# maturk/dn-splatter

Hardware: NVIDIA H100
Metric: rendered Mpix/s (fwd+bwd, RGB+depth+normal) (higher is better)
Workload: dtype f32

## Files before the change

### dn_splatter_b200/csrc/ssim.cu

```cuda
#include "common.cuh"

namespace {

constexpr int SS_R = 5;
constexpr int SS_T = 16;
constexpr int SS_H = SS_T + 2 * SS_R;
constexpr int SS_P = 28;
constexpr int SS_C = 3;
constexpr int SS_NT = 256;

__constant__ float c_win[11] = {1.028380357e-03f, 7.598758209e-03f, 3.600077331e-02f, 1.093606874e-01f, 2.130055279e-01f,
                                2.660117149e-01f, 2.130055279e-01f, 1.093606874e-01f, 3.600077331e-02f, 7.598758209e-03f,
                                1.028380357e-03f};

template <bool U8>
__device__ __forceinline__ float ld_gt(const void* img, size_t idx) {
  return U8 ? __fmul_rn((float)((const uint8_t*)img)[idx], 1.0f / 255.0f) : ((const float*)img)[idx];
}

template <int NQ_IN, int NQ_OUT, int NC, typename Make>
__device__ __forceinline__ void hpass(float (*s_in)[SS_C][SS_H][SS_P], float (*s_mid)[SS_C][SS_H][SS_T], int tid, Make make) {
  constexpr int items = NC * SS_H * (SS_T / 2);
  for (int it = tid; it < items; it += SS_NT) {
    const int seg = it % (SS_T / 2), r = (it / (SS_T / 2)) % SS_H, c = it / ((SS_T / 2) * SS_H);
    float in[NQ_IN][12];
#pragma unroll
    for (int q = 0; q < NQ_IN; ++q) {
      const float2* p = reinterpret_cast<const float2*>(&s_in[q][c][r][2 * seg]);
#pragma unroll
      for (int k = 0; k < 6; ++k) { const float2 v = p[k]; in[q][2 * k] = v.x; in[q][2 * k + 1] = v.y; }
    }
    float acc[NQ_OUT][2];
#pragma unroll
    for (int q = 0; q < NQ_OUT; ++q) acc[q][0] = acc[q][1] = 0.f;
#pragma unroll
    for (int k = 0; k < 12; ++k) {
      float v[NQ_OUT];
      float src[NQ_IN];
#pragma unroll
      for (int q = 0; q < NQ_IN; ++q) src[q] = in[q][k];
      make(src, v);
#pragma unroll
      for (int q = 0; q < NQ_OUT; ++q) {
        if (k < 11) acc[q][0] += c_win[k] * v[q];
        if (k > 0) acc[q][1] += c_win[k - 1] * v[q];
      }
    }
#pragma unroll
    for (int q = 0; q < NQ_OUT; ++q) *reinterpret_cast<float2*>(&s_mid[q][c][r][2 * seg]) = make_float2(acc[q][0], acc[q][1]);
  }
}

template <int NQ>
__device__ __forceinline__ void vpass(float (*s_mid)[SS_C][SS_H][SS_T], int c, int col, int g, float out[NQ][4]) {
#pragma unroll
  for (int q = 0; q < NQ; ++q) {
    float v[14];
#pragma unroll
    for (int j = 0; j < 14; ++j) v[j] = s_mid[q][c][4 * g + j][col];
#pragma unroll
    for (int o = 0; o < 4; ++o) {
      float acc = 0.f;
#pragma unroll
      for (int k = 0; k < 11; ++k) acc += c_win[k] * v[o + k];
      out[q][o] = acc;
    }
  }
}

template <bool U8, bool L1, int NC>
__global__ void __launch_bounds__(SS_NT) ssim_fwd_kernel(const float* __restrict__ x, const void* __restrict__ y, int H, int W,
                                                        int C, int c0, float* __restrict__ dmaps, float* __restrict__ sum_out) {
  __shared__ __align__(16) float s_in[2][SS_C][SS_H][SS_P];
  __shared__ __align__(16) float s_mid[5][SS_C][SS_H][SS_T];
  __shared__ float red[SS_NT / 32];
  __shared__ float red_l1[SS_NT / 32];
  const int tid = threadIdx.x;
  constexpr int nc = NC;
  const int i0 = blockIdx.y * SS_T - SS_R, j0 = blockIdx.x * SS_T - SS_R;
  for (int e = tid; e < SS_H * SS_H * NC; e += SS_NT) {
    const int c = e % NC, q = (e / NC) % SS_H, r = e / (NC * SS_H);
    const int i = i0 + r, j = j0 + q;
    float xv = 0.f, yv = 0.f;
    if (i >= 0 && i < H && j >= 0 && j < W) {
      const size_t p = ((size_t)i * W + j) * C + c0 + c;
      xv = x[p];
      yv = ld_gt<U8>(y, p);
    }
    s_in[0][c][r][q] = xv;
    s_in[1][c][r][q] = yv;
  }
  __syncthreads();
  hpass<2, 5, NC>(s_in, s_mid, tid, [](const float* s, float* v) {
    v[0] = s[0]; v[1] = s[1]; v[2] = s[0] * s[0]; v[3] = s[1] * s[1]; v[4] = s[0] * s[1];
  });
  __syncthreads();
  float ssum = 0.f, lsum = 0.f;
  if (tid < nc * SS_T * 4) {
    const int col = tid % SS_T, g = (tid / SS_T) % 4, c = tid / (SS_T * 4);
    float f[5][4];
    vpass<5>(s_mid, c, col, g, f);
    const int j = blockIdx.x * SS_T + col;
    const size_t n = (size_t)H * W * C;
#pragma unroll
    for (int o = 0; o < 4; ++o) {
      const int i = blockIdx.y * SS_T + 4 * g + o;
      const bool interior = (i >= SS_R) && (i < H - SS_R) && (j >= SS_R) && (j < W - SS_R);
      float s = 0.f, d_mu = 0.f, d_xx = 0.f, d_xy = 0.f;
      if (interior) {
        const float C1 = 0.0001f, C2 = 0.0009f;
        const float mx = f[0][o], my = f[1][o];
        const float sx = f[2][o] - mx * mx, sy = f[3][o] - my * my, sxy = f[4][o] - mx * my;
        const float A1 = 2.f * mx * my + C1, A2 = 2.f * sxy + C2, B1 = mx * mx + my * my + C1, B2 = sx + sy + C2;
        const float inv = 1.0f / (B1 * B2);
        s = A1 * A2 * inv;
        d_xx = -s / B2;
        d_xy = 2.f * A1 * inv;
        d_mu = 2.f * my * (A2 - A1) * inv - 2.f * mx * s / B1 + 2.f * mx * s / B2;
      }
      if (i < H && j < W) {
        const size_t p = ((size_t)i * W + j) * C + c0 + c;
        dmaps[p] = d_mu; dmaps[n + p] = d_xx; dmaps[2 * n + p] = d_xy;
        if (L1) lsum += fabsf(s_in[0][c][4 * g + o + SS_R][col + SS_R] - s_in[1][c][4 * g + o + SS_R][col + SS_R]);
      }
      ssum += s;
    }
  }
  ssum = warp_sum(ssum);
  if (L1) lsum = warp_sum(lsum);
  if ((tid & 31) == 0) { red[tid >> 5] = ssum; if (L1) red_l1[tid >> 5] = lsum; }
  __syncthreads();
  if (tid == 0) {
    float t = 0.f, tl = 0.f;
#pragma unroll
    for (int w = 0; w < SS_NT / 32; ++w) { t += red[w]; if (L1) tl += red_l1[w]; }
    if (t != 0.f) atomicAdd(sum_out, t);
    if (L1 && tl != 0.f) atomicAdd(sum_out + 1, tl);
  }
}

__global__ void photometric_finish_kernel(float* out, float lambda, float inv_count_ssim, float inv_count_l1) {
  out[2] = (1.0f - lambda) * (out[1] * inv_count_l1) + lambda * (1.0f - out[0] * inv_count_ssim);
}

template <bool U8, int NC>
__global__ void __launch_bounds__(SS_NT) ssim_bwd_kernel(const float* __restrict__ x, const void* __restrict__ y, int H, int W,
                                                        int C, int c0, const float* __restrict__ dmaps, const float* v_mean,
                                                        float w_ssim, float w_l1, float* __restrict__ v_x) {
  __shared__ __align__(16) float s_in[3][SS_C][SS_H][SS_P];
  __shared__ __align__(16) float s_mid[3][SS_C][SS_H][SS_T];
  const int tid = threadIdx.x;
  constexpr int nc = NC;
  const int i0 = blockIdx.y * SS_T - SS_R, j0 = blockIdx.x * SS_T - SS_R;
  const size_t n = (size_t)H * W * C;
  for (int e = tid; e < SS_H * SS_H * NC; e += SS_NT) {
    const int c = e % NC, q = (e / NC) % SS_H, r = e / (NC * SS_H);
    const int i = i0 + r, j = j0 + q;
    float a = 0.f, b = 0.f, d = 0.f;
    if (i >= 0 && i < H && j >= 0 && j < W) {
      const size_t p = ((size_t)i * W + j) * C + c0 + c;
      a = dmaps[p]; b = dmaps[n + p]; d = dmaps[2 * n + p];
    }
    s_in[0][c][r][q] = a; s_in[1][c][r][q] = b; s_in[2][c][r][q] = d;
  }
  __syncthreads();
  hpass<3, 3, NC>(s_in, s_mid, tid, [](const float* s, float* v) { v[0] = s[0]; v[1] = s[1]; v[2] = s[2]; });
  __syncthreads();
  if (tid < nc * SS_T * 4) {
    const int col = tid % SS_T, g = (tid / SS_T) % 4, c = tid / (SS_T * 4);
    float f[3][4];
    vpass<3>(s_mid, c, col, g, f);
    const int j = blockIdx.x * SS_T + col;
    const float count = (float)(H - 2 * SS_R) * (float)(W - 2 * SS_R) * (float)C;
    const float vm = v_mean ? __ldg(v_mean) : 1.0f;
    const float gsc = vm * w_ssim / count;
    const float gl1 = vm * w_l1 / ((float)H * (float)W * (float)C);
#pragma unroll
    for (int o = 0; o < 4; ++o) {
      const int i = blockIdx.y * SS_T + 4 * g + o;
      if (i < H && j < W) {
        const size_t p = ((size_t)i * W + j) * C + c0 + c;
        const float xv = x[p], yv = ld_gt<U8>(y, p);
        const float d = xv - yv;
        v_x[p] = gsc * (f[0][o] + 2.f * xv * f[1][o] + yv * f[2][o]) + gl1 * ((d > 0.f) ? 1.f : ((d < 0.f) ? -1.f : 0.f));
      }
    }
  }
}

}

template <bool L1>
static int launch_ssim_fwd(const float* pred, const void* gt, int gt_is_u8, int H, int W, int C, float* dmaps, float* out, cudaStream_t s) {
  const dim3 grid((W + SS_T - 1) / SS_T, (H + SS_T - 1) / SS_T, 1);
  for (int c0 = 0; c0 < C; c0 += SS_C) {
    const int nc = C - c0 < SS_C ? C - c0 : SS_C;
#define DNR_SSIM_FWD(U8, NC) ssim_fwd_kernel<U8, L1, NC><<<grid, SS_NT, 0, s>>>(pred, gt, H, W, C, c0, dmaps, out)
    if (gt_is_u8) { if (nc == 3) DNR_SSIM_FWD(true, 3); else if (nc == 2) DNR_SSIM_FWD(true, 2); else DNR_SSIM_FWD(true, 1); }
    else { if (nc == 3) DNR_SSIM_FWD(false, 3); else if (nc == 2) DNR_SSIM_FWD(false, 2); else DNR_SSIM_FWD(false, 1); }
#undef DNR_SSIM_FWD
    DNR_CHECK_LAUNCH();
  }
  return 0;
}

static int launch_ssim_bwd(const float* pred, const void* gt, int gt_is_u8, int H, int W, int C, const float* dmaps, const float* v,
                           float w_ssim, float w_l1, float* v_pred, cudaStream_t s) {
  const dim3 grid((W + SS_T - 1) / SS_T, (H + SS_T - 1) / SS_T, 1);
  for (int c0 = 0; c0 < C; c0 += SS_C) {
    const int nc = C - c0 < SS_C ? C - c0 : SS_C;
#define DNR_SSIM_BWD(U8, NC) ssim_bwd_kernel<U8, NC><<<grid, SS_NT, 0, s>>>(pred, gt, H, W, C, c0, dmaps, v, w_ssim, w_l1, v_pred)
    if (gt_is_u8) { if (nc == 3) DNR_SSIM_BWD(true, 3); else if (nc == 2) DNR_SSIM_BWD(true, 2); else DNR_SSIM_BWD(true, 1); }
    else { if (nc == 3) DNR_SSIM_BWD(false, 3); else if (nc == 2) DNR_SSIM_BWD(false, 2); else DNR_SSIM_BWD(false, 1); }
#undef DNR_SSIM_BWD
    DNR_CHECK_LAUNCH();
  }
  return 0;
}

extern "C" int dnr_ssim_fwd_ex(const float* pred, const void* gt, int32_t gt_is_u8, int32_t H, int32_t W, int32_t C, float* dmaps,
                               float* sum_out, void* stream) {
  if (!pred || !gt || !dmaps || !sum_out) return DNR_E_NULL;
  if (H <= 2 * SS_R || W <= 2 * SS_R || C <= 0) return DNR_E_SIZE;
  cudaStream_t s = (cudaStream_t)stream;
  DNR_CUDA(cudaMemsetAsync(sum_out, 0, sizeof(float), s));
  return launch_ssim_fwd<false>(pred, gt, gt_is_u8, H, W, C, dmaps, sum_out, s);
}

extern "C" int dnr_photometric_fwd(const float* pred, const void* gt, int32_t gt_is_u8, int32_t H, int32_t W, int32_t C,
                                   float ssim_lambda, float* dmaps, float* out, void* stream) {
  if (!pred || !gt || !dmaps || !out) return DNR_E_NULL;
  if (H <= 2 * SS_R || W <= 2 * SS_R || C <= 0) return DNR_E_SIZE;
  cudaStream_t s = (cudaStream_t)stream;
  DNR_CUDA(cudaMemsetAsync(out, 0, 3 * sizeof(float), s));
  if (const int rc = launch_ssim_fwd<true>(pred, gt, gt_is_u8, H, W, C, dmaps, out, s)) return rc;
  photometric_finish_kernel<<<1, 1, 0, s>>>(out, ssim_lambda, 1.0f / ((float)(H - 2 * SS_R) * (float)(W - 2 * SS_R) * (float)C),
                                            1.0f / ((float)H * (float)W * (float)C));
  DNR_CHECK_LAUNCH();
  return 0;
}

extern "C" int dnr_photometric_bwd(const float* pred, const void* gt, int32_t gt_is_u8, int32_t H, int32_t W, int32_t C,
                                   float ssim_lambda, const float* dmaps, const float* v_main, float* v_pred, void* stream) {
  if (!pred || !gt || !dmaps || !v_pred) return DNR_E_NULL;
  if (H <= 2 * SS_R || W <= 2 * SS_R || C <= 0) return DNR_E_SIZE;
  return launch_ssim_bwd(pred, gt, gt_is_u8, H, W, C, dmaps, v_main, -ssim_lambda, 1.0f - ssim_lambda, v_pred, (cudaStream_t)stream);
}

extern "C" int dnr_ssim_bwd_ex(const float* pred, const void* gt, int32_t gt_is_u8, int32_t H, int32_t W, int32_t C,
                               const float* dmaps, const float* v_mean, float* v_pred, void* stream) {
  if (!pred || !gt || !dmaps || !v_pred) return DNR_E_NULL;
  if (H <= 2 * SS_R || W <= 2 * SS_R || C <= 0) return DNR_E_SIZE;
  return launch_ssim_bwd(pred, gt, gt_is_u8, H, W, C, dmaps, v_mean, 1.0f, 0.0f, v_pred, (cudaStream_t)stream);
}

extern "C" int dnr_ssim_fwd(const float* pred, const float* gt, int32_t H, int32_t W, int32_t C, float* dmaps, float* sum_out,
                            void* stream) {
  return dnr_ssim_fwd_ex(pred, gt, 0, H, W, C, dmaps, sum_out, stream);
}

extern "C" int dnr_ssim_bwd(const float* pred, const float* gt, int32_t H, int32_t W, int32_t C, const float* dmaps,
                            const float* v_mean, float* v_pred, void* stream) {
  return dnr_ssim_bwd_ex(pred, gt, 0, H, W, C, dmaps, v_mean, v_pred, stream);
}
```

### dn_splatter_b200/regularization_strategy.py

```python
from __future__ import annotations

import ctypes as C
from abc import abstractmethod
from typing import Optional

import torch
import torch.nn as nn
import torch.nn.functional as F
from torch import Tensor

from . import _lib as L
from .losses import DepthLoss, DepthLossType, NormalLoss, NormalLossType

_FUSED_DEPTH = {DepthLossType.EdgeAwareLogL1: 1, DepthLossType.LogL1: 2, DepthLossType.L1: 3, DepthLossType.MSE: 4}


def _stream() -> C.c_void_p:
    return C.c_void_p(torch.cuda.current_stream().cuda_stream)


def _shared_holder(*tensors):
    from .rasterize import raster_holder

    hs = [raster_holder(t) for t in tensors if t is not None]
    if not hs or any(h is None for h in hs) or any(h is not hs[0] for h in hs):
        return None
    return hs[0]


class _FusedDNLoss(torch.autograd.Function):

    @staticmethod
    def forward(ctx, pred_depth, pred_normal, gt_depth, gt_normal, gt_img, depth_type: int, depth_lambda: float,
                depth_tolerance: float, use_normal: bool, holder=None, edge_image=None):
        lib = L.load()
        ref = pred_depth if pred_depth is not None else pred_normal
        if ref.device.type != "cuda":
            raise L.DnrError("DNRegularization: the fused regulariser needs CUDA tensors (no CPU path)")
        if depth_type:
            H, W = pred_depth.shape[0], pred_depth.shape[1]
        else:
            H, W = pred_normal.shape[0], pred_normal.shape[1]
        dev = ref.device

        def prep(t, keep_u8=False):
            if t is None:
                return None
            if keep_u8 and t.dtype == torch.uint8:
                return t.detach().to(device=dev).contiguous()
            return t.detach().to(device=dev, dtype=torch.float32).contiguous()

        pd, pn, gd, gi = prep(pred_depth), prep(pred_normal), prep(gt_depth), prep(gt_img)
        gn = prep(gt_normal, keep_u8=True)
        ei = prep(edge_image, keep_u8=True)
        flags = 0
        if gn is not None and gn.dtype == torch.uint8:
            flags |= L.LOSS_NORMAL_U8
        if ei is not None:
            assert ei.dtype == torch.uint8, "edge_image is the raw uint8 image"
            flags |= L.LOSS_EDGE_FROM_IMAGE | L.LOSS_IMG_U8
        partials = torch.empty(12, dtype=torch.float32, device=dev)
        a = L.DnrArgs()
        a.width, a.height = W, H
        a.depth_loss_type, a.use_normal_loss = int(depth_type), int(bool(use_normal))
        a.depth_lambda, a.depth_tolerance = float(depth_lambda), float(depth_tolerance)
        a.loss_flags = flags
        for k, t in dict(out_depth=pd, out_normal=pn, gt_depth=gd, gt_normal=gn, gt_rgb=gi, gt_image=ei,
                         loss_partials=partials).items():
            setattr(a, k, None if t is None else t.data_ptr())
        L.check(lib.dnr_loss_fwd(C.byref(a), _stream()), "dnr_loss_fwd")
        ctx.keep = (pd, pn, gd, gn, gi, ei, partials)
        ctx.fwd_stream = torch.cuda.current_stream()
        ctx.cfg = (W, H, int(depth_type), int(bool(use_normal)), float(depth_lambda), float(depth_tolerance), flags)
        ctx.shapes = (None if pred_depth is None else pred_depth.shape, None if pred_normal is None else pred_normal.shape)
        ctx.holder = holder
        return partials[11].clone()

    @staticmethod
    def backward(ctx, v):
        with torch.cuda.stream(ctx.fwd_stream):
            return _FusedDNLoss._backward(ctx, v)

    @staticmethod
    def _backward(ctx, v):
        lib = L.load()
        pd, pn, gd, gn, gi, ei, partials = ctx.keep
        W, H, depth_type, use_normal, lam, tol, flags = ctx.cfg
        v = v.detach().to(torch.float32).contiguous()
        none9 = (None,) * 9
        if ctx.holder is not None:
            from .rasterize import zero_token

            ctx.holder.setdefault("deferred", {})["reg"] = dict(
                depth_type=depth_type, use_normal=use_normal, depth_lambda=lam, depth_tolerance=tol, gt_depth=gd,
                gt_normal=gn if use_normal else None, gt_rgb=gi, edge_image=ei, loss_partials=partials, v=v)
            vd = zero_token(pd.view(ctx.shapes[0])) if (depth_type and ctx.needs_input_grad[0]) else None
            vn = zero_token(pn.view(ctx.shapes[1])) if (use_normal and ctx.needs_input_grad[1]) else None
            return (vd, vn) + none9
        a = L.DnrArgs()
        a.width, a.height = W, H
        a.depth_loss_type, a.use_normal_loss, a.depth_lambda, a.depth_tolerance = depth_type, use_normal, lam, tol
        a.loss_flags = flags
        for k, t in dict(out_depth=pd, out_normal=pn, gt_depth=gd, gt_normal=gn, gt_rgb=gi, gt_image=ei,
                         loss_partials=partials, v_loss=v).items():
            setattr(a, k, None if t is None else t.data_ptr())
        vd = torch.empty(ctx.shapes[0], dtype=torch.float32, device=v.device) if (depth_type and ctx.needs_input_grad[0]) else None
        vn = torch.empty(ctx.shapes[1], dtype=torch.float32, device=v.device) if (use_normal and ctx.needs_input_grad[1]) else None
        if vd is not None or vn is not None:
            L.check(lib.dnr_loss_bwd(C.byref(a), None if vd is None else vd.data_ptr(),
                                     None if vn is None else vn.data_ptr(), _stream()), "dnr_loss_bwd")
        return (vd, vn) + none9


class _ScaleLoss(torch.autograd.Function):

    @staticmethod
    def forward(ctx, scales):
        lib = L.load()
        if scales.device.type != "cuda":
            raise L.DnrError("scale loss: CUDA tensor required (no CPU path)")
        s = scales.detach().float().contiguous()
        out = torch.empty(1, dtype=torch.float32, device=s.device)
        L.check(lib.dnr_scale_loss_fwd(s.data_ptr(), s.shape[0], out.data_ptr(), _stream()), "dnr_scale_loss_fwd")
        ctx.s = s
        ctx.fwd_stream = torch.cuda.current_stream()
        return out[0].clone()

    @staticmethod
    def backward(ctx, v):
        with torch.cuda.stream(ctx.fwd_stream):
            return _ScaleLoss._backward(ctx, v)

    @staticmethod
    def _backward(ctx, v):
        lib = L.load()
        s = ctx.s
        v = v.detach().float().contiguous()
        g = torch.empty_like(s)
        L.check(lib.dnr_scale_loss_bwd(s.data_ptr(), s.shape[0], v.data_ptr(), g.data_ptr(), _stream()),
                "dnr_scale_loss_bwd")
        return g


class FusedL1(torch.autograd.Function):

    @staticmethod
    def forward(ctx, pred, gt, holder=None):
        lib = L.load()
        if pred.device.type != "cuda" or gt.device != pred.device:
            raise L.DnrError("FusedL1 needs CUDA tensors on one device (no CPU path)")
        p = pred.detach().float().contiguous()
        g = gt.detach().contiguous()
        if g.dtype != torch.uint8:
            g = g.float()
        assert g.numel() == p.numel(), "pred / gt size mismatch"
        out = torch.empty(1, dtype=torch.float32, device=p.device)
        L.check(lib.dnr_l1_fwd(p.data_ptr(), g.data_ptr(), p.numel(), int(g.dtype == torch.uint8), out.data_ptr(), _stream()),
                "dnr_l1_fwd")
        ctx.keep = (p, g)
        ctx.shape = pred.shape
        ctx.fwd_stream = torch.cuda.current_stream()
        ctx.holder = holder
        return out[0].clone()

    @staticmethod
    def backward(ctx, v):
        with torch.cuda.stream(ctx.fwd_stream):
            return FusedL1._backward(ctx, v)

    @staticmethod
    def _backward(ctx, v):
        lib = L.load()
        p, g = ctx.keep
        v = v.detach().float().contiguous()
        if ctx.holder is not None:
            from .rasterize import zero_token

            ctx.holder.setdefault("deferred", {})["l1"] = dict(gt=g, v=v)
            return zero_token(p.view(ctx.shape)), None, None
        vp = torch.empty_like(p)
        L.check(lib.dnr_l1_bwd(p.data_ptr(), g.data_ptr(), p.numel(), int(g.dtype == torch.uint8), v.data_ptr(), vp.data_ptr(),
                               _stream()), "dnr_l1_bwd")
        return vp.view(ctx.shape), None, None


class FusedSSIM(torch.autograd.Function):

    @staticmethod
    def forward(ctx, pred, gt):
        lib = L.load()
        if pred.device.type != "cuda" or gt.device != pred.device:
            raise L.DnrError("FusedSSIM needs CUDA tensors on one device (no CPU path)")
        p = pred.detach().float().contiguous()
        g = gt.detach().contiguous()
        if g.dtype != torch.uint8:
            g = g.float()
        assert p.dim() == 3 and p.shape == g.shape, "pred / gt must both be [H,W,C]"
        H, W, Cn = p.shape
        dmaps = torch.empty((3, H, W, Cn), dtype=torch.float32, device=p.device)
        out = torch.empty(1, dtype=torch.float32, device=p.device)
        L.check(lib.dnr_ssim_fwd_ex(p.data_ptr(), g.data_ptr(), int(g.dtype == torch.uint8), H, W, Cn, dmaps.data_ptr(),
                                    out.data_ptr(), _stream()), "dnr_ssim_fwd_ex")
        ctx.keep = (p, g, dmaps)
        ctx.fwd_stream = torch.cuda.current_stream()
        return out[0] / float((H - 10) * (W - 10) * Cn)

    @staticmethod
    def backward(ctx, v):
        with torch.cuda.stream(ctx.fwd_stream):
            lib = L.load()
            p, g, dmaps = ctx.keep
            v = v.detach().float().contiguous()
            vp = torch.empty_like(p)
            H, W, Cn = p.shape
            L.check(lib.dnr_ssim_bwd_ex(p.data_ptr(), g.data_ptr(), int(g.dtype == torch.uint8), H, W, Cn, dmaps.data_ptr(),
                                        v.data_ptr(), vp.data_ptr(), _stream()), "dnr_ssim_bwd_ex")
            return vp, None


class FusedPhotometric(torch.autograd.Function):

    @staticmethod
    def forward(ctx, pred, gt, ssim_lambda: float):
        lib = L.load()
        if pred.device.type != "cuda" or gt.device != pred.device:
            raise L.DnrError("FusedPhotometric needs CUDA tensors on one device (no CPU path)")
        p = pred.detach().float().contiguous()
        g = gt.detach().contiguous()
        if g.dtype != torch.uint8:
            g = g.float()
        assert p.dim() == 3 and p.shape == g.shape, "pred / gt must both be [H,W,C]"
        H, W, Cn = p.shape
        dmaps = torch.empty((3, H, W, Cn), dtype=torch.float32, device=p.device)
        out = torch.empty(3, dtype=torch.float32, device=p.device)
        L.check(lib.dnr_photometric_fwd(p.data_ptr(), g.data_ptr(), int(g.dtype == torch.uint8), H, W, Cn, float(ssim_lambda),
                                        dmaps.data_ptr(), out.data_ptr(), _stream()), "dnr_photometric_fwd")
        ctx.keep = (p, g, dmaps)
        ctx.lam = float(ssim_lambda)
        ctx.fwd_stream = torch.cuda.current_stream()
        return out[2].clone()

    @staticmethod
    def backward(ctx, v):
        with torch.cuda.stream(ctx.fwd_stream):
            lib = L.load()
            p, g, dmaps = ctx.keep
            v = v.detach().float().contiguous()
            vp = torch.empty_like(p)
            H, W, Cn = p.shape
            L.check(lib.dnr_photometric_bwd(p.data_ptr(), g.data_ptr(), int(g.dtype == torch.uint8), H, W, Cn, ctx.lam,
                                            dmaps.data_ptr(), v.data_ptr(), vp.data_ptr(), _stream()), "dnr_photometric_bwd")
            return vp, None, None


def u8_to_float(img: Tensor, divisor: float = 255.0, clamp_min: float = 0.0) -> Tensor:
    src = img.contiguous()
    dst = torch.empty(src.shape, dtype=torch.float32, device=src.device)
    L.check(L.load().dnr_u8_to_f32(src.data_ptr(), src.numel(), float(divisor), float(clamp_min), dst.data_ptr(), _stream()),
            "dnr_u8_to_f32")
    return dst


class RegularizationStrategy(nn.Module):

    def __init__(self, **kwargs):
        super().__init__()
        self.device_indicator_param = nn.Parameter(torch.empty(0))

    @property
    def device(self):
        return self.device_indicator_param.device

    @abstractmethod
    def get_loss(self, **kwargs):
        """Loss"""

    def forward(self, **kwargs):
        return self.get_loss(**kwargs)

    def get_scale_loss(self, scales):
        return _ScaleLoss.apply(scales)


class DNRegularization(RegularizationStrategy):

    def __init__(self, depth_tolerance: float = 0.1,
                 depth_loss_type: Optional[DepthLossType] = DepthLossType.EdgeAwareLogL1,
                 depth_lambda: float = 0.2, normal_lambda: float = 0.1):
        super().__init__()
        self.depth_tolerance = depth_tolerance
        self.depth_loss_type = depth_loss_type
        self.depth_loss = DepthLoss(self.depth_loss_type)
        self.depth_lambda = depth_lambda
        self.normal_loss_type = NormalLossType.L1
        self.normal_loss = NormalLoss(self.normal_loss_type)
        self.normal_smooth_loss_type = NormalLossType.Smooth
        self.normal_smooth_loss = NormalLoss(self.normal_smooth_loss_type)
        self.normal_lambda = normal_lambda

    def _fusable(self, with_depth: bool) -> bool:
        return (not with_depth) or self.depth_loss_type in _FUSED_DEPTH

    fuse_backward = True
    """Hand the backward of the fused terms to dnr_raster_bwd when the maps are direct raster outputs."""

    def get_loss(self, pred_depth, gt_depth, pred_normal, gt_normal, **kwargs):
        with_depth = self.depth_loss is not None
        with_normal = self.normal_loss is not None
        if self._fusable(with_depth) and (with_depth or with_normal):
            if with_depth and gt_depth is None:
                raise TypeError("use_depth_loss is set but the batch holds no depth (reference: '>' on NoneType)")
            dtype = _FUSED_DEPTH[self.depth_loss_type] if with_depth else 0
            gt_img = kwargs.get("gt_img") if dtype == 1 else None
            edge_image = None
            if dtype == 1 and gt_img is None:
                raise KeyError("gt_img")
            if gt_img is not None and gt_img.dtype == torch.uint8:
                gt_img, edge_image = None, gt_img
            pd, pn = (pred_depth if with_depth else None), (pred_normal if with_normal else None)
            holder = _shared_holder(pd, pn) if self.fuse_backward else None
            loss = _FusedDNLoss.apply(pd, pn, gt_depth if with_depth else None, gt_normal if with_normal else None, gt_img,
                                      dtype, self.depth_lambda, self.depth_tolerance, with_normal, holder, edge_image)
        else:
            if gt_normal is not None and gt_normal.dtype == torch.uint8:
                gt_normal = u8_to_float(gt_normal) if gt_normal.is_cuda else gt_normal.float() / 255.0
            if kwargs.get("gt_img") is not None and kwargs["gt_img"].dtype == torch.uint8:
                gi = kwargs["gt_img"]
                kwargs["gt_img"] = u8_to_float(gi, 255.0, 10 / 255.0) if gi.is_cuda else (gi.float() / 255.0).clamp(min=10 / 255.0)
            loss = 0.0
            if with_depth:
                loss = loss + self.get_depth_loss(pred_depth, gt_depth, **kwargs)
            if with_normal:
                loss = loss + self.get_normal_loss(pred_normal, gt_normal, **kwargs)
        return loss + self.get_scale_loss(scales=kwargs["scales"])

    def get_depth_loss(self, pred_depth, gt_depth, **kwargs):
        valid = gt_depth > self.depth_tolerance
        if self.depth_loss_type in _FUSED_DEPTH:
            gt_img = kwargs.get("gt_img") if self.depth_loss_type == DepthLossType.EdgeAwareLogL1 else None
            return _FusedDNLoss.apply(pred_depth, None, gt_depth, None, gt_img, _FUSED_DEPTH[self.depth_loss_type],
                                      self.depth_lambda, self.depth_tolerance, False)
        if self.depth_loss_type == DepthLossType.PearsonDepth:
            n_valid = valid.sum()
            glob = (self.depth_loss(pred_depth, gt_depth.float()) * n_valid) / n_valid
            local = (DepthLoss(DepthLossType.LocalPearsonDepthLoss)(pred_depth, gt_depth.float()) * n_valid) / n_valid
            d = glob + self.depth_lambda * local
            return d + self.depth_lambda * d
        d = self.depth_loss(pred_depth[valid], gt_depth[valid].float())
        return d + self.depth_lambda * d

    def get_normal_loss(self, pred_normal, gt_normal, **kwargs):
        return _FusedDNLoss.apply(None, pred_normal, None, gt_normal, None, 0, 0.0, self.depth_tolerance, True)


def mean_angular_error(pred: Tensor, gt: Tensor) -> Tensor:
    return torch.arccos(torch.clip((gt * pred).sum(0), -1.0, 1.0))


def find_edges(im: Tensor, threshold: float = 0.01, dilation_itr: int = 1) -> Tensor:
    c = im.shape[0]
    lap = torch.tensor([[0, 1, 0], [1, -4, 1], [0, 1, 0]], dtype=torch.float32, device=im.device)
    lap = lap[None, None].expand(c, 1, 3, 3).contiguous()
    box = torch.ones(c, 1, 3, 3, dtype=torch.float32, device=im.device)
    edges = (F.conv2d((1.0 / (im.float() + 1e-6))[None], lap, padding=1, groups=c) > threshold).float()
    dil = edges
    for _ in range(dilation_itr):
        dil = F.conv2d(dil if c == 1 else edges, box, padding=1, groups=c)
    return dil[0] > 0.0


class AGSMeshRegularization(RegularizationStrategy):

    def __init__(self, depth_tolerance: float = 0.1,
                 depth_loss_type: Optional[DepthLossType] = DepthLossType.EdgeAwareLogL1, depth_lambda: float = 0.2,
                 normal_lambda: float = 0.1, normal_mask_steps: int = 15000, depth_mask_steps: int = 7000):
        super().__init__()
        self.depth_tolerance, self.depth_loss_type = depth_tolerance, depth_loss_type
        self.depth_loss = DepthLoss(self.depth_loss_type)
        self.depth_lambda = depth_lambda
        self.normal_loss_type = NormalLossType.L1
        self.normal_loss = NormalLoss(self.normal_loss_type)
        self.normal_smooth_loss_type = NormalLossType.Smooth
        self.normal_smooth_loss = NormalLoss(self.normal_smooth_loss_type)
        self.normal_lambda = normal_lambda
        self.normal_mask_steps, self.depth_mask_steps = normal_mask_steps, depth_mask_steps
        self.step = 0

    def get_loss(self, step, pred_depth, gt_depth, surf_normal, gt_normal, pred_normal, confidence_map, **kwargs):
        d = self.get_depth_loss(step=step, pred_depth=pred_depth, gt_depth=gt_depth, confidence_map=confidence_map, **kwargs)
        n = self.get_normal_loss(step, surf_normal, gt_normal, pred_normal)
        return d + n + self.get_scale_loss(scales=kwargs["scales"])

    def get_scale_loss(self, scales):
        return torch.min(torch.exp(scales), dim=1, keepdim=True)[0].mean()

    def get_depth_loss(self, step, pred_depth, gt_depth, confidence_map, **kwargs):
        if step >= 7000:
            gt_depth = torch.where(confidence_map > 0, gt_depth, torch.zeros_like(gt_depth))
        mask = gt_depth > self.depth_tolerance
        if self.depth_loss_type == DepthLossType.EdgeAwareLogL1:
            return self.depth_loss(pred_depth, gt_depth.float(), kwargs["gt_img"], mask) * self.depth_lambda
        return self.depth_loss(pred_depth[mask], gt_depth[mask]) * self.depth_lambda

    def get_normal_loss(self, step, surf_normal, gt_normal, pred_normal):
        lam = self.normal_lambda if step > 7000 else 0.0
        if step < self.normal_mask_steps:
            keep = ~find_edges(gt_normal)
            l1 = self.normal_loss(surf_normal[keep], gt_normal[keep]) * lam
        else:
            conf = ~(mean_angular_error(surf_normal, gt_normal) > 0.1)
            l1 = self.normal_loss(surf_normal[:, conf], gt_normal[:, conf]) * lam
        return l1 + self.normal_loss(pred_normal, gt_normal) * lam
```

Baseline: 771.3.

## Restructure SSIM kernels: vertical-first column pass in registers, wider tiles, staged coalesced stores

```diff
diff --git a/dn_splatter_b200/csrc/ssim.cu b/dn_splatter_b200/csrc/ssim.cu
--- a/dn_splatter_b200/csrc/ssim.cu
+++ b/dn_splatter_b200/csrc/ssim.cu
@@ -3,108 +3,115 @@
 namespace {
 
 constexpr int SS_R = 5;
-constexpr int SS_T = 16;
-constexpr int SS_H = SS_T + 2 * SS_R;
-constexpr int SS_P = 28;
+constexpr int SS_NT = 256;
+constexpr int SS_TH = 16;
+constexpr int SS_NR = SS_TH + 2 * SS_R;
+constexpr int SS_TF = 192;
+constexpr int SS_B = 4;
 constexpr int SS_C = 3;
-constexpr int SS_NT = 256;
 
 __constant__ float c_win[11] = {1.028380357e-03f, 7.598758209e-03f, 3.600077331e-02f, 1.093606874e-01f, 2.130055279e-01f,
                                 2.660117149e-01f, 2.130055279e-01f, 1.093606874e-01f, 3.600077331e-02f, 7.598758209e-03f,
                                 1.028380357e-03f};
 
+template <int NC>
+struct SsTile {
+  static constexpr int TW = SS_TF / NC;
+  static constexpr int HW = TW + 2 * SS_R;
+  static constexpr int F = HW * NC;
+  static constexpr int HP = (HW + 3) & ~3;
+  static constexpr int ITEMS = (TW / SS_B) * NC * SS_TH;
+  static_assert(F <= SS_NT && TW % SS_B == 0 && ITEMS % SS_NT == 0 && SS_TH * SS_TF % SS_NT == 0, "tile shape");
+  static constexpr size_t smem(int nq) { return sizeof(float) * ((size_t)nq * SS_TH * NC * HP + 3 * SS_TH * SS_TF); }
+};
+
 template <bool U8>
 __device__ __forceinline__ float ld_gt(const void* img, size_t idx) {
   return U8 ? __fmul_rn((float)((const uint8_t*)img)[idx], 1.0f / 255.0f) : ((const float*)img)[idx];
 }
 
-template <int NQ_IN, int NQ_OUT, int NC, typename Make>
-__device__ __forceinline__ void hpass(float (*s_in)[SS_C][SS_H][SS_P], float (*s_mid)[SS_C][SS_H][SS_T], int tid, Make make) {
-  constexpr int items = NC * SS_H * (SS_T / 2);
-  for (int it = tid; it < items; it += SS_NT) {
-    const int seg = it % (SS_T / 2), r = (it / (SS_T / 2)) % SS_H, c = it / ((SS_T / 2) * SS_H);
-    float in[NQ_IN][12];
-#pragma unroll
-    for (int q = 0; q < NQ_IN; ++q) {
-      const float2* p = reinterpret_cast<const float2*>(&s_in[q][c][r][2 * seg]);
-#pragma unroll
-      for (int k = 0; k < 6; ++k) { const float2 v = p[k]; in[q][2 * k] = v.x; in[q][2 * k + 1] = v.y; }
-    }
-    float acc[NQ_OUT][2];
-#pragma unroll
-    for (int q = 0; q < NQ_OUT; ++q) acc[q][0] = acc[q][1] = 0.f;
-#pragma unroll
-    for (int k = 0; k < 12; ++k) {
-      float v[NQ_OUT];
-      float src[NQ_IN];
-#pragma unroll
-      for (int q = 0; q < NQ_IN; ++q) src[q] = in[q][k];
-      make(src, v);
-#pragma unroll
-      for (int q = 0; q < NQ_OUT; ++q) {
-        if (k < 11) acc[q][0] += c_win[k] * v[q];
-        if (k > 0) acc[q][1] += c_win[k - 1] * v[q];
+template <int NC, int NIN, int NQ, typename Make>
+__device__ __forceinline__ void vpass(const float (&in)[SS_NR][NIN], Make make, float* s_mid, int f) {
+  using T = SsTile<NC>;
+  float* col = s_mid + (f % NC) * T::HP + f / NC;
+  float acc[SS_TH][NQ];
+#pragma unroll
+  for (int i = 0; i < SS_NR; ++i) {
+    float v[NQ];
+    make(in[i], v);
+#pragma unroll
+    for (int k = 0; k < 2 * SS_R + 1; ++k) {
+      const int o = i - k;
+      if (o >= 0 && o < SS_TH) {
+#pragma unroll
+        for (int q = 0; q < NQ; ++q) acc[o][q] = (k == 0) ? c_win[0] * v[q] : acc[o][q] + c_win[k] * v[q];
       }
     }
-#pragma unroll
-    for (int q = 0; q < NQ_OUT; ++q) *reinterpret_cast<float2*>(&s_mid[q][c][r][2 * seg]) = make_float2(acc[q][0], acc[q][1]);
-  }
-}
-
-template <int NQ>
-__device__ __forceinline__ void vpass(float (*s_mid)[SS_C][SS_H][SS_T], int c, int col, int g, float out[NQ][4]) {
-#pragma unroll
-  for (int q = 0; q < NQ; ++q) {
-    float v[14];
-#pragma unroll
-    for (int j = 0; j < 14; ++j) v[j] = s_mid[q][c][4 * g + j][col];
-#pragma unroll
-    for (int o = 0; o < 4; ++o) {
-      float acc = 0.f;
-#pragma unroll
-      for (int k = 0; k < 11; ++k) acc += c_win[k] * v[o + k];
-      out[q][o] = acc;
-    }
+    if (i >= 2 * SS_R) {
+#pragma unroll
+      for (int q = 0; q < NQ; ++q) col[(q * SS_TH + i - 2 * SS_R) * NC * T::HP] = acc[i - 2 * SS_R][q];
+    }
+  }
+}
+
+__device__ __forceinline__ void hfilt4(const float* p, float out[SS_B]) {
+  const float4 a = *reinterpret_cast<const float4*>(p), b = *reinterpret_cast<const float4*>(p + 4),
+               c = *reinterpret_cast<const float4*>(p + 8);
+  const float2 d = *reinterpret_cast<const float2*>(p + 12);
+  const float v[14] = {a.x, a.y, a.z, a.w, b.x, b.y, b.z, b.w, c.x, c.y, c.z, c.w, d.x, d.y};
+#pragma unroll
+  for (int o = 0; o < SS_B; ++o) {
+    float acc = c_win[0] * v[o];
+#pragma unroll
+    for (int k = 1; k < 2 * SS_R + 1; ++k) acc += c_win[k] * v[o + k];
+    out[o] = acc;
   }
 }
 
 template <bool U8, bool L1, int NC>
-__global__ void __launch_bounds__(SS_NT) ssim_fwd_kernel(const float* __restrict__ x, const void* __restrict__ y, int H, int W,
-                                                        int C, int c0, float* __restrict__ dmaps, float* __restrict__ sum_out) {
-  __shared__ __align__(16) float s_in[2][SS_C][SS_H][SS_P];
-  __shared__ __align__(16) float s_mid[5][SS_C][SS_H][SS_T];
-  __shared__ float red[SS_NT / 32];
-  __shared__ float red_l1[SS_NT / 32];
+__global__ void __launch_bounds__(SS_NT, 2) ssim_fwd_kernel(const float* __restrict__ x, const void* __restrict__ y, int H, int W,
+                                                           int C, int c0, float* __restrict__ dmaps, float* __restrict__ sum_out) {
+  using T = SsTile<NC>;
+  extern __shared__ __align__(16) float s_dyn[];
+  float* s_mid = s_dyn;
+  float* s_out = s_dyn + 5 * SS_TH * NC * T::HP;
+  __shared__ float red[2][SS_NT / 32];
   const int tid = threadIdx.x;
-  constexpr int nc = NC;
-  const int i0 = blockIdx.y * SS_T - SS_R, j0 = blockIdx.x * SS_T - SS_R;
-  for (int e = tid; e < SS_H * SS_H * NC; e += SS_NT) {
-    const int c = e % NC, q = (e / NC) % SS_H, r = e / (NC * SS_H);
-    const int i = i0 + r, j = j0 + q;
-    float xv = 0.f, yv = 0.f;
-    if (i >= 0 && i < H && j >= 0 && j < W) {
-      const size_t p = ((size_t)i * W + j) * C + c0 + c;
-      xv = x[p];
-      yv = ld_gt<U8>(y, p);
-    }
-    s_in[0][c][r][q] = xv;
-    s_in[1][c][r][q] = yv;
-  }
-  __syncthreads();
-  hpass<2, 5, NC>(s_in, s_mid, tid, [](const float* s, float* v) {
-    v[0] = s[0]; v[1] = s[1]; v[2] = s[0] * s[0]; v[3] = s[1] * s[1]; v[4] = s[0] * s[1];
-  });
-  __syncthreads();
+  const int i0 = blockIdx.y * SS_TH, j0 = blockIdx.x * T::TW;
   float ssum = 0.f, lsum = 0.f;
-  if (tid < nc * SS_T * 4) {
-    const int col = tid % SS_T, g = (tid / SS_T) % 4, c = tid / (SS_T * 4);
-    float f[5][4];
-    vpass<5>(s_mid, c, col, g, f);
-    const int j = blockIdx.x * SS_T + col;
-    const size_t n = (size_t)H * W * C;
-#pragma unroll
-    for (int o = 0; o < 4; ++o) {
-      const int i = blockIdx.y * SS_T + 4 * g + o;
+  if (tid < T::F) {
+    const int j = j0 - SS_R + tid / NC;
+    const bool col_ok = j >= 0 && j < W;
+    const size_t base = (size_t)(j < 0 ? 0 : j) * C + c0 + tid % NC, pitch = (size_t)W * C;
+    float in[SS_NR][2];
+#pragma unroll
+    for (int i = 0; i < SS_NR; ++i) {
+      const int ig = i0 - SS_R + i;
+      const bool ok = col_ok && ig >= 0 && ig < H;
+      const size_t p = base + (size_t)(ok ? ig : 0) * pitch;
+      in[i][0] = ok ? x[p] : 0.f;
+      in[i][1] = ok ? ld_gt<U8>(y, p) : 0.f;
+    }
+    if (L1 && tid / NC >= SS_R && tid / NC < SS_R + T::TW && col_ok) {
+#pragma unroll
+      for (int i = SS_R; i < SS_R + SS_TH; ++i)
+        if (i0 - SS_R + i < H) lsum += fabsf(in[i][0] - in[i][1]);
+    }
+    vpass<NC, 2, 5>(in, [](const float* s, float* v) {
+      v[0] = s[0]; v[1] = s[1]; v[2] = s[0] * s[0]; v[3] = s[1] * s[1]; v[4] = s[0] * s[1];
+    }, s_mid, tid);
+  }
+  __syncthreads();
+#pragma unroll 1
+  for (int it = tid; it < T::ITEMS; it += SS_NT) {
+    const int pb = it % (T::TW / SS_B), c = (it / (T::TW / SS_B)) % NC, r = it / ((T::TW / SS_B) * NC);
+    float f[5][SS_B];
+#pragma unroll
+    for (int q = 0; q < 5; ++q) hfilt4(s_mid + ((q * SS_TH + r) * NC + c) * T::HP + pb * SS_B, f[q]);
+    const int i = i0 + r;
+#pragma unroll
+    for (int o = 0; o < SS_B; ++o) {
+      const int j = j0 + pb * SS_B + o;
       const bool interior = (i >= SS_R) && (i < H - SS_R) && (j >= SS_R) && (j < W - SS_R);
       float s = 0.f, d_mu = 0.f, d_xx = 0.f, d_xy = 0.f;
       if (interior) {
@@ -118,22 +125,29 @@
         d_xy = 2.f * A1 * inv;
         d_mu = 2.f * my * (A2 - A1) * inv - 2.f * mx * s / B1 + 2.f * mx * s / B2;
       }
-      if (i < H && j < W) {
-        const size_t p = ((size_t)i * W + j) * C + c0 + c;
-        dmaps[p] = d_mu; dmaps[n + p] = d_xx; dmaps[2 * n + p] = d_xy;
-        if (L1) lsum += fabsf(s_in[0][c][4 * g + o + SS_R][col + SS_R] - s_in[1][c][4 * g + o + SS_R][col + SS_R]);
-      }
+      const int e = r * SS_TF + (pb * SS_B + o) * NC + c;
+      s_out[e] = d_mu; s_out[SS_TH * SS_TF + e] = d_xx; s_out[2 * SS_TH * SS_TF + e] = d_xy;
       ssum += s;
+    }
+  }
+  __syncthreads();
+  const size_t n = (size_t)H * W * C;
+#pragma unroll 4
+  for (int e = tid; e < SS_TH * SS_TF; e += SS_NT) {
+    const int r = e / SS_TF, fo = e % SS_TF, i = i0 + r, j = j0 + fo / NC;
+    if (i < H && j < W) {
+      const size_t p = ((size_t)i * W + j) * C + c0 + fo % NC;
+      dmaps[p] = s_out[e]; dmaps[n + p] = s_out[SS_TH * SS_TF + e]; dmaps[2 * n + p] = s_out[2 * SS_TH * SS_TF + e];
     }
   }
   ssum = warp_sum(ssum);
   if (L1) lsum = warp_sum(lsum);
-  if ((tid & 31) == 0) { red[tid >> 5] = ssum; if (L1) red_l1[tid >> 5] = lsum; }
+  if ((tid & 31) == 0) { red[0][tid >> 5] = ssum; red[1][tid >> 5] = lsum; }
   __syncthreads();
   if (tid == 0) {
     float t = 0.f, tl = 0.f;
 #pragma unroll
-    for (int w = 0; w < SS_NT / 32; ++w) { t += red[w]; if (L1) tl += red_l1[w]; }
+    for (int w = 0; w < SS_NT / 32; ++w) { t += red[0][w]; tl += red[1][w]; }
     if (t != 0.f) atomicAdd(sum_out, t);
     if (L1 && tl != 0.f) atomicAdd(sum_out + 1, tl);
   }
@@ -144,76 +158,112 @@
 }
 
 template <bool U8, int NC>
-__global__ void __launch_bounds__(SS_NT) ssim_bwd_kernel(const float* __restrict__ x, const void* __restrict__ y, int H, int W,
-                                                        int C, int c0, const float* __restrict__ dmaps, const float* v_mean,
-                                                        float w_ssim, float w_l1, float* __restrict__ v_x) {
-  __shared__ __align__(16) float s_in[3][SS_C][SS_H][SS_P];
-  __shared__ __align__(16) float s_mid[3][SS_C][SS_H][SS_T];
+__global__ void __launch_bounds__(SS_NT, 2) ssim_bwd_kernel(const float* __restrict__ x, const void* __restrict__ y, int H, int W,
+                                                           int C, int c0, const float* __restrict__ dmaps, const float* v_mean,
+                                                           float w_ssim, float w_l1, float* __restrict__ v_x) {
+  using T = SsTile<NC>;
+  extern __shared__ __align__(16) float s_dyn[];
+  float* s_mid = s_dyn;
+  float* s_out = s_dyn + 3 * SS_TH * NC * T::HP;
   const int tid = threadIdx.x;
-  constexpr int nc = NC;
-  const int i0 = blockIdx.y * SS_T - SS_R, j0 = blockIdx.x * SS_T - SS_R;
+  const int i0 = blockIdx.y * SS_TH, j0 = blockIdx.x * T::TW;
   const size_t n = (size_t)H * W * C;
-  for (int e = tid; e < SS_H * SS_H * NC; e += SS_NT) {
-    const int c = e % NC, q = (e / NC) % SS_H, r = e / (NC * SS_H);
-    const int i = i0 + r, j = j0 + q;
-    float a = 0.f, b = 0.f, d = 0.f;
-    if (i >= 0 && i < H && j >= 0 && j < W) {
-      const size_t p = ((size_t)i * W + j) * C + c0 + c;
-      a = dmaps[p]; b = dmaps[n + p]; d = dmaps[2 * n + p];
-    }
-    s_in[0][c][r][q] = a; s_in[1][c][r][q] = b; s_in[2][c][r][q] = d;
-  }
-  __syncthreads();
-  hpass<3, 3, NC>(s_in, s_mid, tid, [](const float* s, float* v) { v[0] = s[0]; v[1] = s[1]; v[2] = s[2]; });
-  __syncthreads();
-  if (tid < nc * SS_T * 4) {
-    const int col = tid % SS_T, g = (tid / SS_T) % 4, c = tid / (SS_T * 4);
-    float f[3][4];
-    vpass<3>(s_mid, c, col, g, f);
-    const int j = blockIdx.x * SS_T + col;
-    const float count = (float)(H - 2 * SS_R) * (float)(W - 2 * SS_R) * (float)C;
-    const float vm = v_mean ? __ldg(v_mean) : 1.0f;
-    const float gsc = vm * w_ssim / count;
-    const float gl1 = vm * w_l1 / ((float)H * (float)W * (float)C);
-#pragma unroll
-    for (int o = 0; o < 4; ++o) {
-      const int i = blockIdx.y * SS_T + 4 * g + o;
-      if (i < H && j < W) {
-        const size_t p = ((size_t)i * W + j) * C + c0 + c;
-        const float xv = x[p], yv = ld_gt<U8>(y, p);
-        const float d = xv - yv;
-        v_x[p] = gsc * (f[0][o] + 2.f * xv * f[1][o] + yv * f[2][o]) + gl1 * ((d > 0.f) ? 1.f : ((d < 0.f) ? -1.f : 0.f));
-      }
-    }
-  }
-}
-
+  if (tid < T::F) {
+    const int j = j0 - SS_R + tid / NC;
+    const bool col_ok = j >= 0 && j < W;
+    const size_t base = (size_t)(j < 0 ? 0 : j) * C + c0 + tid % NC, pitch = (size_t)W * C;
+    float in[SS_NR][3];
+#pragma unroll
+    for (int i = 0; i < SS_NR; ++i) {
+      const int ig = i0 - SS_R + i;
+      const bool ok = col_ok && ig >= 0 && ig < H;
+      const size_t p = base + (size_t)(ok ? ig : 0) * pitch;
+      in[i][0] = ok ? dmaps[p] : 0.f;
+      in[i][1] = ok ? dmaps[n + p] : 0.f;
+      in[i][2] = ok ? dmaps[2 * n + p] : 0.f;
+    }
+    vpass<NC, 3, 3>(in, [](const float* s, float* v) { v[0] = s[0]; v[1] = s[1]; v[2] = s[2]; }, s_mid, tid);
+  }
+  __syncthreads();
+#pragma unroll 1
+  for (int it = tid; it < T::ITEMS; it += SS_NT) {
+    const int pb = it % (T::TW / SS_B), c = (it / (T::TW / SS_B)) % NC, r = it / ((T::TW / SS_B) * NC);
+    float f[3][SS_B];
+#pragma unroll
+    for (int q = 0; q < 3; ++q) hfilt4(s_mid + ((q * SS_TH + r) * NC + c) * T::HP + pb * SS_B, f[q]);
+#pragma unroll
+    for (int o = 0; o < SS_B; ++o) {
+      const int e = r * SS_TF + (pb * SS_B + o) * NC + c;
+      s_out[e] = f[0][o]; s_out[SS_TH * SS_TF + e] = f[1][o]; s_out[2 * SS_TH * SS_TF + e] = f[2][o];
+    }
+  }
+  __syncthreads();
+  const float count = (float)(H - 2 * SS_R) * (float)(W - 2 * SS_R) * (float)C;
+  const float vm = v_mean ? __ldg(v_mean) : 1.0f;
+  const float gsc = vm * w_ssim / count;
+  const float gl1 = vm * w_l1 / ((float)H * (float)W * (float)C);
+#pragma unroll 4
+  for (int e = tid; e < SS_TH * SS_TF; e += SS_NT) {
+    const int r = e / SS_TF, fo = e % SS_TF, i = i0 + r, j = j0 + fo / NC;
+    if (i < H && j < W) {
+      const size_t p = ((size_t)i * W + j) * C + c0 + fo % NC;
+      const float xv = x[p], yv = ld_gt<U8>(y, p);
+      const float d = xv - yv;
+      v_x[p] = gsc * (s_out[e] + 2.f * xv * s_out[SS_TH * SS_TF + e] + yv * s_out[2 * SS_TH * SS_TF + e]) +
+               gl1 * ((d > 0.f) ? 1.f : ((d < 0.f) ? -1.f : 0.f));
+    }
+  }
+}
+
+}
+
+template <bool U8, bool L1, int NC>
+static int launch_ssim_fwd_nc(const float* pred, const void* gt, int H, int W, int C, int c0, float* dmaps, float* out, cudaStream_t s) {
+  using T = SsTile<NC>;
+  static const cudaError_t attr = cudaFuncSetAttribute(ssim_fwd_kernel<U8, L1, NC>, cudaFuncAttributeMaxDynamicSharedMemorySize,
+                                                       (int)T::smem(5));
+  if (attr != cudaSuccess) return (int)attr;
+  const dim3 grid((W + T::TW - 1) / T::TW, (H + SS_TH - 1) / SS_TH, 1);
+  ssim_fwd_kernel<U8, L1, NC><<<grid, SS_NT, T::smem(5), s>>>(pred, gt, H, W, C, c0, dmaps, out);
+  DNR_CHECK_LAUNCH();
+  return 0;
+}
+
+template <bool U8, int NC>
+static int launch_ssim_bwd_nc(const float* pred, const void* gt, int H, int W, int C, int c0, const float* dmaps, const float* v,
+                              float w_ssim, float w_l1, float* v_pred, cudaStream_t s) {
+  using T = SsTile<NC>;
+  static const cudaError_t attr = cudaFuncSetAttribute(ssim_bwd_kernel<U8, NC>, cudaFuncAttributeMaxDynamicSharedMemorySize,
+                                                       (int)T::smem(3));
+  if (attr != cudaSuccess) return (int)attr;
+  const dim3 grid((W + T::TW - 1) / T::TW, (H + SS_TH - 1) / SS_TH, 1);
+  ssim_bwd_kernel<U8, NC><<<grid, SS_NT, T::smem(3), s>>>(pred, gt, H, W, C, c0, dmaps, v, w_ssim, w_l1, v_pred);
+  DNR_CHECK_LAUNCH();
+  return 0;
 }
 
 template <bool L1>
 static int launch_ssim_fwd(const float* pred, const void* gt, int gt_is_u8, int H, int W, int C, float* dmaps, float* out, cudaStream_t s) {
-  const dim3 grid((W + SS_T - 1) / SS_T, (H + SS_T - 1) / SS_T, 1);
   for (int c0 = 0; c0 < C; c0 += SS_C) {
     const int nc = C - c0 < SS_C ? C - c0 : SS_C;
-#define DNR_SSIM_FWD(U8, NC) ssim_fwd_kernel<U8, L1, NC><<<grid, SS_NT, 0, s>>>(pred, gt, H, W, C, c0, dmaps, out)
-    if (gt_is_u8) { if (nc == 3) DNR_SSIM_FWD(true, 3); else if (nc == 2) DNR_SSIM_FWD(true, 2); else DNR_SSIM_FWD(true, 1); }
-    else { if (nc == 3) DNR_SSIM_FWD(false, 3); else if (nc == 2) DNR_SSIM_FWD(false, 2); else DNR_SSIM_FWD(false, 1); }
+#define DNR_SSIM_FWD(U8, NC) launch_ssim_fwd_nc<U8, L1, NC>(pred, gt, H, W, C, c0, dmaps, out, s)
+    const int rc = gt_is_u8 ? (nc == 3 ? DNR_SSIM_FWD(true, 3) : nc == 2 ? DNR_SSIM_FWD(true, 2) : DNR_SSIM_FWD(true, 1))
+                            : (nc == 3 ? DNR_SSIM_FWD(false, 3) : nc == 2 ? DNR_SSIM_FWD(false, 2) : DNR_SSIM_FWD(false, 1));
 #undef DNR_SSIM_FWD
-    DNR_CHECK_LAUNCH();
+    if (rc) return rc;
   }
   return 0;
 }
 
 static int launch_ssim_bwd(const float* pred, const void* gt, int gt_is_u8, int H, int W, int C, const float* dmaps, const float* v,
                            float w_ssim, float w_l1, float* v_pred, cudaStream_t s) {
-  const dim3 grid((W + SS_T - 1) / SS_T, (H + SS_T - 1) / SS_T, 1);
   for (int c0 = 0; c0 < C; c0 += SS_C) {
     const int nc = C - c0 < SS_C ? C - c0 : SS_C;
-#define DNR_SSIM_BWD(U8, NC) ssim_bwd_kernel<U8, NC><<<grid, SS_NT, 0, s>>>(pred, gt, H, W, C, c0, dmaps, v, w_ssim, w_l1, v_pred)
-    if (gt_is_u8) { if (nc == 3) DNR_SSIM_BWD(true, 3); else if (nc == 2) DNR_SSIM_BWD(true, 2); else DNR_SSIM_BWD(true, 1); }
-    else { if (nc == 3) DNR_SSIM_BWD(false, 3); else if (nc == 2) DNR_SSIM_BWD(false, 2); else DNR_SSIM_BWD(false, 1); }
+#define DNR_SSIM_BWD(U8, NC) launch_ssim_bwd_nc<U8, NC>(pred, gt, H, W, C, c0, dmaps, v, w_ssim, w_l1, v_pred, s)
+    const int rc = gt_is_u8 ? (nc == 3 ? DNR_SSIM_BWD(true, 3) : nc == 2 ? DNR_SSIM_BWD(true, 2) : DNR_SSIM_BWD(true, 1))
+                            : (nc == 3 ? DNR_SSIM_BWD(false, 3) : nc == 2 ? DNR_SSIM_BWD(false, 2) : DNR_SSIM_BWD(false, 1));
 #undef DNR_SSIM_BWD
-    DNR_CHECK_LAUNCH();
+    if (rc) return rc;
   }
   return 0;
 }
diff --git a/dn_splatter_b200/regularization_strategy.py b/dn_splatter_b200/regularization_strategy.py
--- a/dn_splatter_b200/regularization_strategy.py
+++ b/dn_splatter_b200/regularization_strategy.py
@@ -11,6 +11,7 @@
 
 from . import _lib as L
 from .losses import DepthLoss, DepthLossType, NormalLoss, NormalLossType
+from .rasterize import _timed
 
 _FUSED_DEPTH = {DepthLossType.EdgeAwareLogL1: 1, DepthLossType.LogL1: 2, DepthLossType.L1: 3, DepthLossType.MSE: 4}
 
@@ -68,7 +69,7 @@
         for k, t in dict(out_depth=pd, out_normal=pn, gt_depth=gd, gt_normal=gn, gt_rgb=gi, gt_image=ei,
                          loss_partials=partials).items():
             setattr(a, k, None if t is None else t.data_ptr())
-        L.check(lib.dnr_loss_fwd(C.byref(a), _stream()), "dnr_loss_fwd")
+        L.check(_timed("loss_fwd", lib.dnr_loss_fwd, C.byref(a), _stream()), "dnr_loss_fwd")
         ctx.keep = (pd, pn, gd, gn, gi, ei, partials)
         ctx.fwd_stream = torch.cuda.current_stream()
         ctx.cfg = (W, H, int(depth_type), int(bool(use_normal)), float(depth_lambda), float(depth_tolerance), flags)
@@ -233,8 +234,8 @@
         H, W, Cn = p.shape
         dmaps = torch.empty((3, H, W, Cn), dtype=torch.float32, device=p.device)
         out = torch.empty(3, dtype=torch.float32, device=p.device)
-        L.check(lib.dnr_photometric_fwd(p.data_ptr(), g.data_ptr(), int(g.dtype == torch.uint8), H, W, Cn, float(ssim_lambda),
-                                        dmaps.data_ptr(), out.data_ptr(), _stream()), "dnr_photometric_fwd")
+        L.check(_timed("photometric_fwd", lib.dnr_photometric_fwd, p.data_ptr(), g.data_ptr(), int(g.dtype == torch.uint8), H, W,
+                       Cn, float(ssim_lambda), dmaps.data_ptr(), out.data_ptr(), _stream()), "dnr_photometric_fwd")
         ctx.keep = (p, g, dmaps)
         ctx.lam = float(ssim_lambda)
         ctx.fwd_stream = torch.cuda.current_stream()
@@ -248,8 +249,8 @@
             v = v.detach().float().contiguous()
             vp = torch.empty_like(p)
             H, W, Cn = p.shape
-            L.check(lib.dnr_photometric_bwd(p.data_ptr(), g.data_ptr(), int(g.dtype == torch.uint8), H, W, Cn, ctx.lam,
-                                            dmaps.data_ptr(), v.data_ptr(), vp.data_ptr(), _stream()), "dnr_photometric_bwd")
+            L.check(_timed("photometric_bwd", lib.dnr_photometric_bwd, p.data_ptr(), g.data_ptr(), int(g.dtype == torch.uint8), H,
+                           W, Cn, ctx.lam, dmaps.data_ptr(), v.data_ptr(), vp.data_ptr(), _stream()), "dnr_photometric_bwd")
             return vp, None, None
 
 
```

New measurement: 794.2, median of 6. 1.03x the previous value.
